# datamicroscopes/common

Measured on AMD Instinct MI355X. Metric: score_value evals/sec, higher is better.
Workload: dtype f32

## Files before the change

common_amd/csrc/abi.cpp:

```cpp
#include <algorithm>
#include <atomic>
#include <cmath>
#include <memory>
#include <mutex>
#include <new>

#include "blocked_post.hpp"
#include "launchers.hpp"
#include "linkage_host.hpp"
#include "row_range.hpp"
#include "splitmerge_math.hpp"

namespace msc {

static thread_local std::string g_last_error;

void set_error(const char *fmt, ...) {
  char buf[1024];
  va_list ap;
  va_start(ap, fmt);
  vsnprintf(buf, sizeof buf, fmt, ap);
  va_end(ap);
  g_last_error = buf;
}
// ... 1627 lines not shown
static uint64_t view_rows(const msc_state *st) {
  return st->sweep_rows_hint ? st->sweep_rows_hint : st->bound_view ? st->bound_view->nrows : 0;
}

static int refresh_fused_tables(msc_state *st) {
  const bool packed = stages_nich(st->tile_path);
  if (!st->fuse_any && !st->nich_blocks_any && !packed) return MSC_OK;
  if (launch_fuse_tables(st->ctx->stream, st->desc_fuse_dev, (int)st->fuse_split, (st->nich_blocks_any || packed) ? (int)st->fuse_nfeat : (int)st->fuse_split, st->kpad))
    return fail(MSC_EHIP, "k_fuse_tables launch failed");
  return MSC_OK;
}

static bool narrow_tail_fits(const msc_state *st) {
  const size_t nich_bytes = (size_t)(st->fuse_nfeat - st->fuse_split) * 64 * sizeof(float);
  return st->tile_narrow_tail_ok && st->K - (st->kpad - kGroupTile) <= kTailMaxGroups &&
         nich_bytes + (size_t)std::max<uint32_t>(1u, st->tail_max_rows) * kTailStride * sizeof(float) <= 64u * 1024u;
}

static int tail_plan(msc_state *st, TailPlan &tp, bool exact = true) {
  tp = TailPlan();
  tp.exact = exact;
  if (!(tp.ok = narrow_tail_fits(st))) return MSC_OK;
  MSC_HIP(grow_retained(st->retired, st->tail_pack, (size_t)st->tail_pack_rows * 64));
  tp.masked_nich = st->tail_masked_nich;
  tp.dm = st->tail_dm;
  tp.max_rows = st->tail_max_rows;
  tp.pack_rows = st->tail_pack_rows;
  tp.pack = st->tail_pack;
  return MSC_OK;
}

static bool gp_beyond_table(const msc_state *st, uint32_t f) {
  if (!st->bound_view || f >= st->bound_cols.size()) return false;
  const uint32_t c = st->bound_cols[f];
  if (is_count_family(st->feats[f].family)) return col_max_of(st, f, st->bound_view, c) >= (long long)kGpMaxTable;
  if (st->feats[f].family == MSC_DM)
    return !st->bound_view->dm_max[c].empty() && dm_max_of(st, f, st->bound_view, c, st->feats[f].dim) >= kGpMaxTable;
  return false;
}

static bool loo_needs_heavy(const msc_state *st) {
  for (uint32_t f = 0; f < st->nfeat; f++) {
    const int fam = st->feats[f].family;
    if ((is_count_family(fam) || fam == MSC_DM) && gp_beyond_table(st, f)) return true;
  }
  return false;
// ... 2438 lines not shown
```

common_amd/csrc/kernels_score.hip:

```cpp
#include <cstdlib>
#include <type_traits>

#include "commit_ops.hpp"
#include "family_math.hpp"
#include "launchers.hpp"
#include "score_block.hpp"

namespace msc {

__global__ __launch_bounds__(256) void k_prepare(const FeatDesc *__restrict__ feats, uint32_t kpad) {
  const uint32_t k = blockIdx.x * 256 + threadIdx.x;
  if (k >= kpad) return;
  prepare_group(feats[blockIdx.y], k, kpad, blockIdx.z, gridDim.z);
}

__global__ __launch_bounds__(256) void k_dm_prepare(const FeatDesc *__restrict__ feats, int f, uint32_t kpad) {
  const FeatDesc fd = feats[f];
  const uint32_t k = blockIdx.x * 256 + threadIdx.x, sub = blockIdx.y;
  if (k >= kpad || fd.dm_meta == nullptr) return;
  const uint32_t first = fd.dm_meta[2 * sub], rows = fd.dm_meta[2 * sub + 1];
  float *t = fd.tab + (size_t)first * kpad + k;
  double a = 0, n = 0;
  if (sub < fd.dim) {
    a = fd.hp[sub];
// ... 890 lines not shown
    hipLaunchKernelGGL(k_loo_own<false>, dim3((unsigned)((nrows + 255) / 256)), dim3(256), 0, stream, feats_dev, nfeat,
                       K, kpad, row0, nrows, z, crp, own);
  return hipGetLastError() == hipSuccess ? 0 : -1;
}

int launch_gp_large_fix(hipStream_t stream, int num_cus, const FeatDesc *feats_dev, int f, uint32_t K,
                        uint32_t kpad, uint64_t row0, uint64_t nrows, const int32_t *z, float *out, uint64_t ld) {
  uint64_t gx = (nrows + 3) / 4;
  const uint64_t cap = (uint64_t)num_cus * 8;
  if (gx > cap) gx = cap;
  hipLaunchKernelGGL(k_gp_large_fix, dim3((unsigned)(gx ? gx : 1)), dim3(256), 0, stream, feats_dev, f, K, kpad,
                     row0, nrows, z, out, ld);
  return hipGetLastError() == hipSuccess ? 0 : -1;
}

const Nich1Shape kNich1Shapes[kNich1NumShapes] = {{4, 2}, {4, 1}, {4, 4}, {4, 6}, {4, 3}, {4, 8}, {4, 5}, {4, 12}};

constexpr int kTailRowsWaves = 8;

__host__ __device__ inline uint32_t tail_table_rows(uint32_t family, uint32_t kind, uint32_t run_clamp, uint32_t dm_rows) {
  return family == MSC_DM ? dm_rows : kind == MSC_KIND_GENERIC ? 0u : run_clamp + 1;
}

__global__ __launch_bounds__(256) void k_tail_pack(const FeatDesc *__restrict__ feats, uint32_t kpad, uint32_t k0,
                                                    float *__restrict__ pack) {
  const int f = blockIdx.x;
  uint32_t off = 0;
  for (int i = 0; i < f; i++) off += tail_table_rows(feats[i].family, feats[i].kind, feats[i].run_clamp, feats[i].dm_rows);
  const FeatDesc &fd = feats[f];
  const uint32_t first_row = is_count_family(fd.family) ? (uint32_t)GP_T0 : 0u, rows = tail_table_rows(fd.family, fd.kind, fd.run_clamp, fd.dm_rows);
  for (uint32_t e = threadIdx.x; e < rows * 64u; e += 256u) {
    const uint32_t r = e >> 6, g = e & 63u;
    pack[(size_t)(off + r) * 64 + g] = fd.tab[(size_t)(first_row + r) * kpad + k0 + g];
  }
}

template <int TGP, bool SPLIT, bool DRAW = false, bool MNICH = false, bool EST = false, bool DMF = false>
__global__ __launch_bounds__(kTailRowsWaves * 64, (MNICH || DMF) ? 2 : 4) void k_score_tail_rows(
    const FeatDesc *__restrict__ feats_g, int nfeat, int nsplit, uint32_t K, uint32_t kpad, uint32_t k0, uint64_t row0,
    uint64_t nrows, int32_t *z, const float *__restrict__ own, const float *__restrict__ crp,
    float *__restrict__ out, uint64_t ld, const float *__restrict__ pack, uint32_t cap_rows, uint32_t kend,
    const uint64_t *__restrict__ rng, uint64_t row_id0, ZeroSpans zero) {
  uint64_t seed = 0, sweep = 0;
  if (DRAW) {
    seed = rng[0];
    sweep = rng[1];
    zero_spans(zero);
  }
  extern __shared__ __attribute__((aligned(16))) float tl[];
  __shared__ __attribute__((aligned(16))) float pr[4][64];
  __shared__ __attribute__((aligned(16))) float c0s[64];
  float *const mhl = tl + (size_t)cap_rows * kTailStride;
  typedef const __attribute__((address_space(4))) FeatDesc *scalar_fd;
  typedef const __attribute__((address_space(4))) float *scalar_f;
  const scalar_fd feats = (scalar_fd)feats_g;
  const int lane = threadIdx.x & 63, wave = __builtin_amdgcn_readfirstlane(threadIdx.x >> 6);
  const bool loo = z != nullptr, pri = crp != nullptr;
  const bool vec_ok = ((ld & 3) == 0) && ((reinterpret_cast<uintptr_t>(out) & 15) == 0);
  const uint64_t rows_per_wg = (uint64_t)kTailRowsWaves * 64;
  const uint64_t nchunks = (nrows + rows_per_wg - 1) / rows_per_wg;
  if (threadIdx.x < 64) {
    float hi = 0.f, lo = 0.f, le0 = 0.f, le1 = 0.f, e0 = 0.f, e1 = 0.f;
    if (pri) {
      hi = crp[k0 + threadIdx.x];
      lo = crp[crp_lo_cnt(kpad) + k0 + threadIdx.x];
      le0 = crp[2 * (size_t)kpad];
      le1 = crp[2 * (size_t)kpad + 1];
      e0 = crp[2 * (size_t)kpad + 2];
      e1 = crp[2 * (size_t)kpad + 3];
    }
    const bool empty = __builtin_isinf(hi);
    pr[0][threadIdx.x] = !pri ? 0.f : empty ? e0 : lo;
    pr[1][threadIdx.x] = !pri ? 0.f : empty ? e1 : lo;
    pr[2][threadIdx.x] = !pri ? -0.f : empty ? le0 : hi;
    pr[3][threadIdx.x] = !pri ? -0.f : empty ? le1 : hi;
    float c0 = 0.f;
    for (int f = nsplit; f < nfeat; f++) {
      c0 += feats_g[f].tab[(size_t)NICH_C0 * kpad + k0 + threadIdx.x];
      mhl[(size_t)(f - nsplit) * 64 + threadIdx.x] = feats_g[f].tab[(size_t)NICH_MU_HI * kpad + k0 + threadIdx.x];
    }
    c0s[threadIdx.x] = c0;
  }
  __syncthreads();
  auto load_value = [&](int f, uint64_t rr) -> uint32_t {
    const int fi = f < nfeat ? f : nfeat - 1;
    const int ct = feats[fi].col_type;
    const void *col = feats[fi].col;
    const bool u8 = ct == MSC_TYPE_B || ct == MSC_TYPE_I8 || ct == MSC_TYPE_U8;
    return u8 ? (uint32_t)reinterpret_cast<const uint8_t *>(col)[rr] : reinterpret_cast<const uint32_t *>(col)[rr];
  };
  for (uint64_t chunk = blockIdx.x; chunk < nchunks; chunk += gridDim.x) {
    const uint64_t r = chunk * rows_per_wg + (uint64_t)wave * 64 + lane;
    const bool has_row = r < nrows;
    const uint64_t rr = row0 + (has_row ? r : 0);
    int gown = (loo && has_row) ? z[r] : -1;
    if ((uint32_t)gown >= K) gown = -1;
    const bool single = pri && gown >= 0 && __builtin_isinf(crp[kpad + gown]);
    const float ownv = gown >= 0 ? own[r] : 0.f;
    const float *prl = pr[single ? 1 : 0];
    float acc[TGP], accn[SPLIT ? TGP : 1];
#pragma unroll
    for (int g = 0; g < TGP; g++) acc[g] = prl[g];
    uint32_t srow = 0, off = 0;
    int stage_end = 0;
    for (int fb = 0; fb < nsplit; fb += 8) {
      uint32_t w0 = load_value(fb, rr), w1 = load_value(fb + 1, rr), w2 = load_value(fb + 2, rr), w3 = load_value(fb + 3, rr),
               w4 = load_value(fb + 4, rr), w5 = load_value(fb + 5, rr), w6 = load_value(fb + 6, rr), w7 = load_value(fb + 7, rr);
#pragma unroll 1
      for (int i = 0; i < 8; i++) {
        const int f = fb + i;
        if (f >= nsplit) break;
        if (f == stage_end) {
          srow += off;
          off = 0;
          uint32_t rows = 0;
          while (stage_end < nsplit) {
            const uint32_t rw = tail_table_rows(feats[stage_end].family, feats[stage_end].kind, feats[stage_end].run_clamp, feats[stage_end].dm_rows);
            if (rows + rw > cap_rows && rows > 0) break;
            rows += rw;
            stage_end++;
          }
          __syncthreads();
          for (uint32_t e = threadIdx.x * 4u; e < rows * 64u; e += kTailRowsWaves * 64u * 4u) {
            const float4 v = *reinterpret_cast<const float4 *>(pack + (size_t)srow * 64 + e);
            float *d = tl + (size_t)(e >> 6) * kTailStride + (e & 63u);
            d[0] = v.x; d[1] = v.y; d[2] = v.z; d[3] = v.w;
          }
          __syncthreads();
        }
        if (DMF && feats[f].family == MSC_DM) {
          const uint32_t dim = feats[f].dim;
          const uint32_t *xr = reinterpret_cast<const uint32_t *>(feats[f].col) + rr * dim;
          const uint32_t *meta = feats[f].dm_meta;
          const uint32_t tot = has_row ? feats[f].dm_tot[rr] : 0u;
          bool dead = !has_row || tot >= kGpMaxTable;
          if (feats[f].mask != nullptr)
            for (uint32_t e = 0; e < dim; e++) dead |= feats[f].mask[rr * dim + e] != 0;
#pragma unroll
          for (int gb = 0; gb < TGP; gb += 16) {
            float hi[16], lo[16];
#pragma unroll
            for (int g = 0; g < 16; g++) hi[g] = lo[g] = 0.f;
#pragma unroll 1
            for (uint32_t st = 0; st <= dim; st++) {
              const uint32_t first_row = meta[2 * st], vcap = meta[2 * st + 1];
              uint32_t v = st < dim ? xr[st] : tot;
              v = (dead || v >= vcap) ? 0u : v;
              const float *b = tl + (size_t)(off + first_row + 2u * v) * kTailStride + gb;
#pragma unroll
              for (int g = 0; g < 16; g++) {
                hi[g] += b[g];
                lo[g] += b[kTailStride + g];
              }
            }
#pragma unroll
            for (int g = 0; g < 16; g++) acc[gb + g] += hi[g] + lo[g];
          }
          off += feats[f].dm_rows;
        } else if (MNICH && feats[f].kind == MSC_KIND_GENERIC) {
          const bool masked = feats[f].mask[rr] != 0;
          const float x = __uint_as_float(w0);
          const scalar_f tab = (scalar_f)(feats[f].tab) + k0;
          typedef float f32x4s __attribute__((ext_vector_type(4)));
          typedef const volatile __attribute__((address_space(4))) f32x4s *scalar_f4;
#pragma unroll
          for (int gb = 0; gb < TGP; gb += 4) {
            const f32x4s mh = *(scalar_f4)(tab + (size_t)NICH_MU_HI * kpad + gb), ml = *(scalar_f4)(tab + (size_t)NICH_MU_LO * kpad + gb),
                         c0 = *(scalar_f4)(tab + (size_t)NICH_C0 * kpad + gb), c1l = *(scalar_f4)(tab + (size_t)NICH_C1LN2 * kpad + gb),
                         c1 = *(scalar_f4)(tab + (size_t)NICH_C1 * kpad + gb), c2 = *(scalar_f4)(tab + (size_t)NICH_C2 * kpad + gb);
#pragma unroll
            for (int j = 0; j < 4; j++) {
              const float e = acc[gb + j] + nich_eval(x, mh[j], ml[j], c0[j], c1l[j], c1[j], c2[j]);
              acc[gb + j] = masked ? acc[gb + j] : e;
            }
            __builtin_amdgcn_sched_barrier(0);
          }
        } else {
          const uint32_t rc = feats[f].run_clamp;
          const int v = (int)w0;
          const uint32_t idx = v < 0 ? 0u : ((uint32_t)v > rc ? rc : (uint32_t)v);
          const float *b = tl + (size_t)(off + idx) * kTailStride;
#pragma unroll
          for (int g = 0; g < TGP; g++) acc[g] += b[g];
          off += rc + 1;
        }
        w0 = w1; w1 = w2; w2 = w3; w3 = w4; w4 = w5; w5 = w6; w6 = w7;
      }
    }
    if (SPLIT) {
#pragma unroll
      for (int g = 0; g < TGP; g++) accn[g] = c0s[g];
    } else if (nsplit < nfeat) {
#pragma unroll
      for (int g = 0; g < TGP; g++) acc[g] += c0s[g];
    }
    bool far = false;
    const bool blocks = nsplit < nfeat && feats[nsplit].nich_info != nullptr;
    for (int fb = nsplit; blocks && fb < nfeat; fb += 8) {
      const uint32_t w0 = load_value(fb, rr), w1 = load_value(fb + 1, rr), w2 = load_value(fb + 2, rr), w3 = load_value(fb + 3, rr),
                     w4 = load_value(fb + 4, rr), w5 = load_value(fb + 5, rr), w6 = load_value(fb + 6, rr), w7 = load_value(fb + 7, rr);
      auto lim = [&](int f) { return feats[f < nfeat ? f : nfeat - 1].nich_info->xlim; };
      far |= !(__builtin_fabsf(__uint_as_float(w0)) <= lim(fb)) | !(__builtin_fabsf(__uint_as_float(w1)) <= lim(fb + 1)) |
             !(__builtin_fabsf(__uint_as_float(w2)) <= lim(fb + 2)) | !(__builtin_fabsf(__uint_as_float(w3)) <= lim(fb + 3)) |
             !(__builtin_fabsf(__uint_as_float(w4)) <= lim(fb + 4)) | !(__builtin_fabsf(__uint_as_float(w5)) <= lim(fb + 5)) |
             !(__builtin_fabsf(__uint_as_float(w6)) <= lim(fb + 6)) | !(__builtin_fabsf(__uint_as_float(w7)) <= lim(fb + 7));
    }
    auto plain_feature = [&](int f, float x) {
      const scalar_f tab = (scalar_f)(feats[f].tab) + k0;
      const float *mhf = mhl + (size_t)(f - nsplit) * 64;
      constexpr int NB = (!SPLIT || TGP <= 32) ? 8 : 4;
      typedef float f32xn __attribute__((ext_vector_type(NB)));
      typedef const volatile __attribute__((address_space(4))) f32xn *scalar_fn;
#pragma unroll
      for (int gb = 0; gb < TGP; gb += NB) {
        const f32xn ml = *(scalar_fn)(tab + (size_t)NICH_MU_LO * kpad + gb), c1l = *(scalar_fn)(tab + (size_t)NICH_C1LN2 * kpad + gb),
                    c1 = *(scalar_fn)(tab + (size_t)NICH_C1 * kpad + gb), c2 = *(scalar_fn)(tab + (size_t)NICH_C2 * kpad + gb);
#pragma unroll
        for (int j = 0; j < NB; j++) {
          float &a = SPLIT ? accn[gb + j] : acc[gb + j];
          a = nich_accum<EST>(a, x, mhf[gb + j], ml[j], c1l[j], c1[j], c2[j]);
        }
        __builtin_amdgcn_sched_barrier(0);
      }
    };
    auto product_block = [&](int f, auto mtag, const float (&x)[4]) {
      constexpr int M = decltype(mtag)::value;
      typedef float f32x4s __attribute__((ext_vector_type(4)));
      typedef const volatile __attribute__((address_space(4))) f32x4s *scalar_f4;
      scalar_f tab[M];
      const float *mhf[M];
#pragma unroll
      for (int j = 0; j < M; j++) {
        tab[j] = (scalar_f)(feats[f + j].tab) + k0;
        mhf[j] = mhl + (size_t)(f + j - nsplit) * 64;
      }
#pragma unroll
      for (int gb = 0; gb < TGP; gb += 4) {
        f32x4s ml[M], sc[M];
#pragma unroll
        for (int j = 0; j < M; j++) {
          ml[j] = *(scalar_f4)(tab[j] + (size_t)NICH_MU_LO * kpad + gb);
          sc[j] = *(scalar_f4)(tab[j] + (size_t)NICH_C2 * kpad + gb);
        }
        const f32x4s c1l = *(scalar_f4)(tab[0] + (size_t)NICH_C1LN2 * kpad + gb);
#pragma unroll
        for (int i = 0; i < 4; i++) {
          float t[M];
#pragma unroll
          for (int j = 0; j < M; j++) t[j] = nich_t(x[j], mhf[j][gb + i], ml[j][i], sc[j][i]);
          float &a = SPLIT ? accn[gb + i] : acc[gb + i];
          a = nich_block_finish<EST>(a, nich_block_product<M>(t), c1l[i]);
        }
        __builtin_amdgcn_sched_barrier(0);
      }
    };
    for (int s0 = nsplit; s0 < nfeat;) {
      const int s1 = (int)feats[s0].grp_end;
      if (blocks) {
#pragma unroll 1
        for (int M = kNichBlock; M >= 2; M--) {
          for (int f = s0; f < s1;) {
            const int len = (int)feats[f].blk_end - f;
            if (len == M && feats[f].nich_info->blk_ok != 0u) {
              const float x[4] = {__uint_as_float(load_value(f, rr)), __uint_as_float(load_value(f + 1, rr)),
                                  __uint_as_float(load_value(f + 2, rr)), __uint_as_float(load_value(f + 3, rr))};
              if (!far) {
                if (M == 2) product_block(f, std::integral_constant<int, 2>(), x);
                else if (M == 3) product_block(f, std::integral_constant<int, 3>(), x);
                else product_block(f, std::integral_constant<int, 4>(), x);
              }
            }
            f += len;
          }
        }
      }
#pragma unroll 1
      for (int f = s0; f < s1; f++) {
        const bool covered = blocks && feats[feats[f].blk_first].nich_info->blk_ok != 0u;
        const float x = __uint_as_float(load_value(f, rr));
        if (far || !covered) plain_feature(f, x);
      }
      s0 = s1;
    }
    const float *prh = pr[single ? 3 : 2];
    if (DRAW) {
      float m = -INFINITY;
#pragma unroll
      for (int g = 0; g < TGP; g++) {
        const float sg = gown == g ? ownv : (SPLIT && nsplit < nfeat ? acc[g] + accn[g] : acc[g]) + prh[g];
        acc[g] = (uint32_t)g < K ? sg : -INFINITY;
        m = fmaxf(m, acc[g]);
      }
      float total = 0.f;
#pragma unroll
      for (int g = 0; g < TGP; g++) {
        acc[g] = __builtin_amdgcn_exp2f((acc[g] - m) * 1.44269504088896340736f);
        total += acc[g];
      }
      const float dart = philox_uniform01(seed, sweep, row_id0 + r) * total;
      float c = 0.f;
      int pick = 0;
// ... 1 lines not shown
      for (int g = 0; g < TGP; g++) {
        c += acc[g];
        pick += c < dart ? 1 : 0;
      }
      if (has_row) z[r] = pick < (int)K ? pick : (int)K - 1;
      continue;
    }
#pragma unroll
    for (int q = 0; q < TGP / 4; q++) {
      float sv[4];
#pragma unroll
      for (int c = 0; c < 4; c++) {
        const int g = 4 * q + c;
        sv[c] = gown == (int)(k0 + g) ? ownv : (SPLIT && nsplit < nfeat ? acc[g] + accn[g] : acc[g]) + prh[g];
      }
      if (has_row) store_row<false>(out, ld, r, k0 + 4 * q, kend, make_float4(sv[0], sv[1], sv[2], sv[3]), vec_ok);
    }
  }
}

template <int TGP, bool SPLIT, bool DRAW, bool MNICH, bool EST, bool DMF = false>
static void launch_tail_rows_m(hipStream_t stream, unsigned grid, size_t lds, const FeatDesc *feats_dev, int nfeat, int nsplit, uint32_t K,
                               uint32_t kpad, uint32_t k0, uint64_t row0, uint64_t nrows, const int32_t *z, const float *own,
                               const float *crp, float *out, uint64_t ld, const float *pack, uint32_t cap_rows, uint32_t kend,
                               const uint64_t *rng, uint64_t row_id0, ZeroSpans zero) {
  static unsigned long long attr_devices = 0;
  if (first_use_on_device(attr_devices))
    (void)hipFuncSetAttribute(reinterpret_cast<const void *>(k_score_tail_rows<TGP, SPLIT, DRAW, MNICH, EST, DMF>), hipFuncAttributeMaxDynamicSharedMemorySize, 64 * 1024);
  hipLaunchKernelGGL((k_score_tail_rows<TGP, SPLIT, DRAW, MNICH, EST, DMF>), (note_kernel(DRAW ? 1 : 0, "k_score_tail_rows<%d, %s, %s, %s, %s, %s>", TGP, tf(SPLIT), tf(DRAW), tf(MNICH), tf(EST), tf(DMF)), dim3(grid)), dim3(kTailRowsWaves * 64), lds, stream, feats_dev, nfeat, nsplit, K, kpad, k0,
                     row0, nrows, const_cast<int32_t *>(z), own, crp, out, ld, pack, cap_rows, kend, rng, row_id0, zero);
}
template <int TGP, bool SPLIT, bool DRAW = false, bool EST = false>
static void launch_tail_rows_t(hipStream_t stream, unsigned grid, size_t lds, int mnich, const FeatDesc *feats_dev, int nfeat, int nsplit, uint32_t K,
                               uint32_t kpad, uint32_t k0, uint64_t row0, uint64_t nrows, const int32_t *z, const float *own,
                               const float *crp, float *out, uint64_t ld, const float *pack, uint32_t cap_rows, uint32_t kend,
                               const uint64_t *rng = nullptr, uint64_t row_id0 = 0, ZeroSpans zero = ZeroSpans()) {
  if (mnich == 2) launch_tail_rows_m<TGP, SPLIT, DRAW, false, EST, true>(stream, grid, lds, feats_dev, nfeat, nsplit, K, kpad, k0, row0, nrows, z, own, crp, out, ld, pack, cap_rows, kend, rng, row_id0, zero);
  else if (mnich) launch_tail_rows_m<TGP, SPLIT, DRAW, true, EST>(stream, grid, lds, feats_dev, nfeat, nsplit, K, kpad, k0, row0, nrows, z, own, crp, out, ld, pack, cap_rows, kend, rng, row_id0, zero);
  else launch_tail_rows_m<TGP, SPLIT, DRAW, false, EST>(stream, grid, lds, feats_dev, nfeat, nsplit, K, kpad, k0, row0, nrows, z, own, crp, out, ld, pack, cap_rows, kend, rng, row_id0, zero);
}

static bool tail_rows_geometry(const TailPlan &tp, int num_cus, int nfeat, int nsplit, uint64_t nrows, uint32_t &cap_rows, size_t &lds,
                               unsigned &grid) {
  if (!tp.ok || (tp.pack_rows > 0 && tp.pack == nullptr)) return false;
  const size_t nich_bytes = (size_t)(nfeat - nsplit) * 64 * sizeof(float);
  const uint32_t fit = (uint32_t)((64u * 1024u - nich_bytes) / (kTailStride * sizeof(float)));
  cap_rows = std::max<uint32_t>(1u, std::min<uint32_t>(tp.pack_rows, std::min<uint32_t>(200u, fit)));
  lds = (size_t)cap_rows * kTailStride * sizeof(float) + nich_bytes;
  const uint64_t rows_wg = (uint64_t)kTailRowsWaves * 64;
  const uint64_t tchunks = (nrows + rows_wg - 1) / rows_wg;
  grid = (unsigned)std::min<uint64_t>(tchunks ? tchunks : 1, (uint64_t)num_cus * 2);
  return true;
}

int launch_sweep_rows(hipStream_t stream, int num_cus, const TailPlan &tp, const FeatDesc *feats_dev, int nfeat, int nsplit, uint32_t K,
                      uint32_t kpad, uint64_t row0, uint64_t nrows, uint64_t row_id0, int32_t *z, const float *own, const float *crp,
                      const uint64_t *rng, ZeroSpans zero) {
  uint32_t cap_rows = 0;
  size_t lds = 0;
  unsigned grid = 0;
  if (K > 64 || crp == nullptr || !tail_rows_geometry(tp, num_cus, nfeat, nsplit, nrows, cap_rows, lds, grid)) return fail(MSC_EHIP, "launch_sweep_rows: K = %u", K);
  if (nsplit > 0) hipLaunchKernelGGL(k_tail_pack, dim3((unsigned)nsplit), dim3(256), 0, stream, feats_dev, kpad, 0u, tp.pack);
  const uint32_t tgp = (K + 15u) / 16u * 16u;
#define MSC_SWEEP_ROWS(T) launch_tail_rows_t<T, false, true, true>(stream, grid, lds, tp.dm ? 2 : tp.masked_nich ? 1 : 0, feats_dev, nfeat, nsplit, K, kpad, 0u, row0, nrows, z, own, crp, nullptr, 0, tp.pack, cap_rows, K, rng, row_id0, zero)
  if (tgp == 16) MSC_SWEEP_ROWS(16);
  else if (tgp == 32)
    launch_tail_rows_t<32, true, true, true>(stream, grid, lds, tp.dm ? 2 : tp.masked_nich ? 1 : 0, feats_dev, nfeat, nsplit, K, kpad, 0u, row0, nrows, z, own, crp, nullptr, 0, tp.pack, cap_rows, K, rng, row_id0, zero);
  else if (tgp == 48) MSC_SWEEP_ROWS(48);
  else MSC_SWEEP_ROWS(64);
#undef MSC_SWEEP_ROWS
  return launch_status("k_score_tail_rows");
}

int launch_score_tail(hipStream_t stream, int num_cus, const TailPlan &tp, const FeatDesc *feats_dev, int nfeat, int nsplit, uint32_t K,
                      uint32_t kpad, uint32_t k0, uint64_t row0, uint64_t nrows, const int32_t *z, const float *own, const float *crp,
                      float *out, uint64_t ld) {
  uint32_t cap_rows = 0;
  size_t lds = 0;
  unsigned grid = 0;
  if (K <= k0 || K - k0 > kTailMaxGroups || !tail_rows_geometry(tp, num_cus, nfeat, nsplit, nrows, cap_rows, lds, grid)) return fail(MSC_EHIP, "launch_score_tail: K = %u", K);
  if (nrows == 0) return 0;
  const uint32_t groups = K - k0, widest = tp.exact ? 32u : 64u, nblk = (groups + widest - 1) / widest;
  const uint32_t blk = ((groups + nblk - 1) / nblk + 15u) / 16u * 16u;
  for (uint32_t kb = k0; kb < K; kb += blk) {
    const uint32_t kend = std::min<uint32_t>(K, kb + blk), tgp = (kend - kb + 15u) / 16u * 16u;
    if (nsplit > 0) hipLaunchKernelGGL(k_tail_pack, dim3((unsigned)nsplit), dim3(256), 0, stream, feats_dev, kpad, kb, tp.pack);
#define MSC_TAIL_ROWS(T, S, E) launch_tail_rows_t<T, S, false, E>(stream, grid, lds, tp.dm ? 2 : tp.masked_nich ? 1 : 0, feats_dev, nfeat, nsplit, K, kpad, kb, row0, nrows, z, own, crp, out, ld, tp.pack, cap_rows, kend)
    if (tp.exact) {
      if (tgp == 16) MSC_TAIL_ROWS(16, true, false);
      else if (tgp == 32) MSC_TAIL_ROWS(32, true, false);
      else MSC_TAIL_ROWS(48, true, false);
    } else {
      if (tgp == 16) MSC_TAIL_ROWS(16, false, true);
      else if (tgp == 32) MSC_TAIL_ROWS(32, true, true);
      else if (tgp == 48) MSC_TAIL_ROWS(48, false, true);
      else MSC_TAIL_ROWS(64, false, true);
    }
#undef MSC_TAIL_ROWS
  }
  return launch_status("k_score_tail_rows");
}

template <bool LOO, bool CRP>
static int launch_score_t(hipStream_t stream, int num_cus, ScorePath path, const TailPlan &narrow_tail, const ScoreShape &shape, const FeatDesc *feats_dev,
                           int nfeat, int nsplit, uint32_t K, uint32_t kpad, uint64_t row0, uint64_t nrows,
                           const int32_t *z, const float *own, const float *crp, float *out, uint64_t ld) {
  const uint32_t ktiles = kpad / kGroupTile;
  if (path == MSC_PATH_NICH1) {
    const bool plain_stores = (shape.nich1 & 0x100) != 0;
    const int nich1_shape = shape.nich1 & 0xff;
// ... 94 lines not shown
```

common_amd/csrc/launchers.hpp:

```cpp
#pragma once
#include <algorithm>

#include "msc_internal.hpp"

namespace msc {

inline bool first_use_on_device(unsigned long long &seen) {
  int dev = 0;
  if (hipGetDevice(&dev) != hipSuccess || dev < 0 || dev > 63) return true;
  const unsigned long long bit = 1ull << dev;
  if (seen & bit) return false;
  seen |= bit;
  return true;
}

struct UnpackFeat {
  void *dst;
  uint8_t *dst_mask;
  uint32_t offset;
  uint32_t mask_offset;
  int32_t src_type, dst_type;
  uint32_t count;
  uint32_t pad;
};
// ... 20 lines not shown
int launch_set_i32(hipStream_t stream, int32_t *dst, int32_t value);
constexpr int kLooRows = 4, kLooThreads = 1024;
int launch_loo_own(hipStream_t stream, bool heavy, bool staged, const FeatDesc *feats_dev, int nfeat, uint32_t K, uint32_t kpad, uint64_t row0,
                   uint64_t nrows, const int32_t *z, const float *crp, float *own);
int launch_gp_large_fix(hipStream_t stream, int num_cus, const FeatDesc *feats_dev, int f, uint32_t K,
                        uint32_t kpad, uint64_t row0, uint64_t nrows, const int32_t *z, float *out, uint64_t ld);
struct Nich1Shape { int q, visits; };
constexpr int kNich1NumShapes = 8;
extern const Nich1Shape kNich1Shapes[kNich1NumShapes];
constexpr uint32_t kTailMaxGroups = 128;
constexpr uint64_t kNarrowMaxRows = 65536;
constexpr uint64_t kTailMinRows = 16384;
constexpr uint32_t kTailStride = 65;
inline double tile_rounds_us(uint64_t workgroups, int num_cus, bool sweep, const PlanCost &pc = PlanCost()) {
  return (sweep ? pc.sweep_round_us : pc.tile_round_us) * (double)((workgroups + (uint64_t)num_cus - 1) / (uint64_t)num_cus);
}
inline double tail_rows_us(uint32_t groups, bool exact, uint64_t nrows, int num_cus, const PlanCost &pc = PlanCost()) {
  const uint32_t widest = exact ? 32u : 64u, nblk = (groups + widest - 1) / widest;
  const uint32_t per = ((groups + nblk - 1) / nblk + 15u) / 16u * 16u;
  const double frac = (double)nrows / (1024.0 * num_cus);
  const double rounds = frac >= 1.0 ? frac : std::max(0.6, 0.4 + 0.6 * frac);
  return (double)nblk * (pc.tail_fixed_us + pc.tail_group_us * per) * rounds;
}
struct TailPlan {
  bool ok = false;
  bool exact = true;
  bool masked_nich = false;
  bool dm = false;
  uint32_t max_rows = 0;
  uint32_t pack_rows = 0;
  float *pack = nullptr;
};
int launch_score_tail(hipStream_t stream, int num_cus, const TailPlan &tp, const FeatDesc *feats_dev, int nfeat, int nsplit, uint32_t K,
                      uint32_t kpad, uint32_t k0, uint64_t row0, uint64_t nrows, const int32_t *z, const float *own, const float *crp,
                      float *out, uint64_t ld);
struct ZeroSpans {
  unsigned long long *a = nullptr;
  size_t na = 0;
  unsigned long long *b = nullptr;
  size_t nb = 0;
};
int launch_sweep_rows(hipStream_t stream, int num_cus, const TailPlan &tp, const FeatDesc *feats_dev, int nfeat, int nsplit, uint32_t K,
                      uint32_t kpad, uint64_t row0, uint64_t nrows, uint64_t row_id0, int32_t *z, const float *own, const float *crp,
                      const uint64_t *rng, ZeroSpans zero);
int launch_score_pair_tail(hipStream_t stream, int num_cus, const FeatDesc *feats_dev, int nfeat, int nsplit, uint32_t K, uint32_t kpad,
                           uint64_t row0, uint64_t nrows, const int32_t *z, const float *own, const float *crp, float *tail, uint64_t ld);
enum class LastTile { tiles, rows, pair };
struct ScoreShape { int wave_rows = 8; bool pair = false; LastTile last = LastTile::tiles; int nich1 = 0; };
int launch_score(hipStream_t stream, int num_cus, ScorePath path, const TailPlan &narrow_tail, const ScoreShape &shape, const FeatDesc *feats_dev, int nfeat, int nsplit,
                 uint32_t K, uint32_t kpad, uint64_t row0, uint64_t nrows, const int32_t *z,
                 const float *own, const float *crp, float *out, uint64_t ld);

void note_kernel(int slot, const char *fmt, ...) __attribute__((format(printf, 2, 3)));
const char *last_kernel(int slot);
// ... 276 lines not shown
```

common_amd/csrc/msc_internal.hpp:

```cpp
#pragma once

#include <hip/hip_runtime.h>

#include <cstdarg>
#include <cstdint>
#include <cstdio>
#include <cstring>
#include <string>
#include <vector>

#include "../../include/microscopes_hip.h"
#include "dev_buf.hpp"
#include "table_validity.hpp"

namespace msc {

constexpr int kWave = 64;
constexpr int kGroupTile = 256;
constexpr unsigned kMaxDDDim = 128;
constexpr int kGrpRows = 128;
constexpr unsigned kGpMaxTable = 1024;
constexpr float kNtFastGbps = 6650.f;

void set_error(const char *fmt, ...);
// ... 432 lines not shown
  uint32_t fuse_nfeat = 0, fuse_split = 0;
  bool fuse_any = false;
  msc::DevBuf<float> fuse_tab;
  msc::DevBuf<msc::FeatDesc> desc_acc_dev;
  std::vector<msc::FeatDesc> desc_acc_host;
  msc::DevBuf<msc::NichPlanInfo> nich_info;
  msc::DevBuf<float> rn_pack;
  msc::DevBuf<msc::NichPos> rn_pos;
  bool nich_blocks_any = false;
  const msc_dataview *bound_view = nullptr;
  uint64_t bound_serial = 0;
  std::vector<uint32_t> bound_cols;
  msc::Retired retired;
  msc::DevBuf<float> scratch;
  msc::DevBuf<float> tail_scores;
  msc::DevBuf<float> own;
  msc::ScorePath tile_path = msc::MSC_PATH_TILE;
  msc::PlanCost plan_cost;
  bool tile_narrow_tail_ok = false;
  uint32_t tail_max_rows = 0, tail_pack_rows = 0;
  bool tail_masked_nich = false;
  bool tail_dm = false;
  msc::DevBuf<float> tail_pack;
  uint32_t loo_staged = 0;
  msc::DevBuf<double> marg_norm;
  msc::DevBuf<float> rows_table;
  msc::DevBuf<uint32_t> colmax_dev;
  msc::DevBuf<uint64_t> rng_dev;
  uint64_t rng_seed = 0, rng_sweep = 0;
  bool rng_valid = false;
  bool rng_bump_pending = false;
  uint64_t rng_next_sweep = 0;
  struct StepGraph {
    hipGraphExec_t exec = nullptr;
    const void *view = nullptr, *z = nullptr;
    uint64_t view_serial = 0, row0 = 0, nrows = 0, row_id0 = 0;
    float alpha = 0.f;
    std::vector<uint32_t> cols;
    msc::TableValidity::Snapshot flags;
    int seen = 0;
    bool disabled = false;
    uint64_t n_eager = 0, n_replayed = 0;
  } step_graph;
  msc::DevBuf<double> niw_qown;
  msc::DevBuf<int32_t> one_z;
  msc::DevBuf<uint32_t> niw_scratch;
// ... 49 lines not shown
```

Before: 1724 billion.

## Precompute compact per-feature tail plan records and narrow packed tables to group width

Measured after the change: 1608 billion. -6.7%, worse.

```diff
diff --git a/common_amd/csrc/abi.cpp b/common_amd/csrc/abi.cpp
--- a/common_amd/csrc/abi.cpp
+++ b/common_amd/csrc/abi.cpp
@@ -1673,6 +1673,8 @@
   tp.exact = exact;
   if (!(tp.ok = narrow_tail_fits(st))) return MSC_OK;
   MSC_HIP(grow_retained(st->retired, st->tail_pack, (size_t)st->tail_pack_rows * 64));
+  MSC_HIP(grow_retained(st->retired, st->tail_feats, tail_plan_words(st->fuse_nfeat, st->fuse_split)));
+  tp.feat_plan = st->tail_feats;
   tp.masked_nich = st->tail_masked_nich;
   tp.dm = st->tail_dm;
   tp.max_rows = st->tail_max_rows;
diff --git a/common_amd/csrc/kernels_score.hip b/common_amd/csrc/kernels_score.hip
--- a/common_amd/csrc/kernels_score.hip
+++ b/common_amd/csrc/kernels_score.hip
@@ -936,16 +936,72 @@
   return family == MSC_DM ? dm_rows : kind == MSC_KIND_GENERIC ? 0u : run_clamp + 1;
 }
 
-__global__ __launch_bounds__(256) void k_tail_pack(const FeatDesc *__restrict__ feats, uint32_t kpad, uint32_t k0,
-                                                    float *__restrict__ pack) {
+constexpr int kTailPlanTile = 1024;
+__device__ void tail_plan_records(const FeatDesc *__restrict__ feats, int nfeat, int nsplit, uint32_t cap_rows, uint32_t *__restrict__ plan) {
+  __shared__ uint32_t rws[kTailPlanTile];
+  TailFeat *const rec = reinterpret_cast<TailFeat *>(plan);
+  TailStage *const stg = reinterpret_cast<TailStage *>(rec + nfeat + kTailFeatPad);
+  const bool blocks = nsplit < nfeat && feats[nsplit].nich_info != nullptr;
+  uint32_t nst = 0, rows = 0, total = 0;
+  for (int base = 0; base < nsplit; base += kTailPlanTile) {
+    const int n = min(nsplit - base, kTailPlanTile);
+    for (int i = threadIdx.x; i < n; i += blockDim.x) {
+      const FeatDesc &fd = feats[base + i];
+      rws[i] = tail_table_rows(fd.family, fd.kind, fd.run_clamp, fd.dm_rows);
+    }
+    __syncthreads();
+    if (threadIdx.x == 0)
+      for (int i = 0; i < n; i++) {
+        const uint32_t rw = rws[i];
+        if (base + i == 0 || (rows + rw > cap_rows && rows > 0)) {
+          if (nst) stg[nst].rows = rows;
+          stg[++nst] = TailStage{(uint32_t)(base + i), total, 0u, 0u};
+          rows = 0;
+          rws[i] = kTailMetaStage;
+        } else {
+          rws[i] = rows;
+        }
+        rows += rw;
+        total += rw;
+      }
+    __syncthreads();
+    for (int i = threadIdx.x; i < n; i += blockDim.x) {
+      const FeatDesc &fd = feats[base + i];
+      const bool u8 = fd.col_type == MSC_TYPE_B || fd.col_type == MSC_TYPE_I8 || fd.col_type == MSC_TYPE_U8;
+      const bool dm = fd.family == MSC_DM, nich = !dm && fd.kind == MSC_KIND_GENERIC;
+      rec[base + i] = TailFeat{fd.col, dm ? fd.dm_rows : fd.run_clamp,
+                               rws[i] | (u8 ? kTailMetaByte : 0u) | (nich ? kTailMetaNich : 0u) | (dm ? kTailMetaDm : 0u), fd.tab, 0u, 0u};
+    }
+    __syncthreads();
+  }
+  if (threadIdx.x == 0) {
+    if (nst) stg[nst].rows = rows;
+    stg[0] = TailStage{nst, blocks ? 1u : 0u, 0u, 0u};
+    if (nst == 1) rec[0].meta &= ~kTailMetaStage;
+  }
+  for (int f = nsplit + (int)threadIdx.x; f < nfeat; f += blockDim.x) {
+    const FeatDesc &fd = feats[f];
+    const bool u8 = fd.col_type == MSC_TYPE_B || fd.col_type == MSC_TYPE_I8 || fd.col_type == MSC_TYPE_U8;
+    uint32_t blk = (fd.blk_end - (uint32_t)f) & kTailBlkLenMask;
+    if (blocks && fd.nich_info->blk_ok != 0u) blk |= kTailBlkOne;
+    if (blocks && feats[fd.blk_first].nich_info->blk_ok != 0u) blk |= kTailBlkCovered;
+    rec[f] = TailFeat{fd.col, __float_as_uint(blocks ? fd.nich_info->xlim : INFINITY), (u8 ? kTailMetaByte : 0u) | kTailMetaNich, fd.tab, fd.grp_end, blk};
+  }
+  __syncthreads();
+  if (nfeat > 0 && threadIdx.x < kTailFeatPad) rec[nfeat + threadIdx.x] = rec[nfeat - 1];
+}
+
+__global__ __launch_bounds__(256) void k_tail_pack(const FeatDesc *__restrict__ feats, int nfeat, int nsplit, uint32_t kpad, uint32_t k0,
+                                                    uint32_t width, uint32_t cap_rows, float *__restrict__ pack, uint32_t *__restrict__ plan) {
   const int f = blockIdx.x;
+  if (f == nsplit) return tail_plan_records(feats, nfeat, nsplit, cap_rows, plan);
   uint32_t off = 0;
   for (int i = 0; i < f; i++) off += tail_table_rows(feats[i].family, feats[i].kind, feats[i].run_clamp, feats[i].dm_rows);
   const FeatDesc &fd = feats[f];
   const uint32_t first_row = is_count_family(fd.family) ? (uint32_t)GP_T0 : 0u, rows = tail_table_rows(fd.family, fd.kind, fd.run_clamp, fd.dm_rows);
   for (uint32_t e = threadIdx.x; e < rows * 64u; e += 256u) {
     const uint32_t r = e >> 6, g = e & 63u;
-    pack[(size_t)(off + r) * 64 + g] = fd.tab[(size_t)(first_row + r) * kpad + k0 + g];
+    if (g < width) pack[(size_t)(off + r) * width + g] = fd.tab[(size_t)(first_row + r) * kpad + k0 + g];
   }
 }
 
@@ -953,21 +1009,36 @@
 __global__ __launch_bounds__(kTailRowsWaves * 64, (MNICH || DMF) ? 2 : 4) void k_score_tail_rows(
     const FeatDesc *__restrict__ feats_g, int nfeat, int nsplit, uint32_t K, uint32_t kpad, uint32_t k0, uint64_t row0,
     uint64_t nrows, int32_t *z, const float *__restrict__ own, const float *__restrict__ crp,
-    float *__restrict__ out, uint64_t ld, const float *__restrict__ pack, uint32_t cap_rows, uint32_t kend,
-    const uint64_t *__restrict__ rng, uint64_t row_id0, ZeroSpans zero) {
+    float *__restrict__ out, uint64_t ld, const float *__restrict__ pack, const uint32_t *__restrict__ plan_g, uint32_t cap_rows,
+    uint32_t kend, const uint64_t *__restrict__ rng, uint64_t row_id0, ZeroSpans zero) {
   uint64_t seed = 0, sweep = 0;
   if (DRAW) {
     seed = rng[0];
     sweep = rng[1];
     zero_spans(zero);
   }
+  constexpr uint32_t kStride = TGP + 1;
   extern __shared__ __attribute__((aligned(16))) float tl[];
   __shared__ __attribute__((aligned(16))) float pr[4][64];
   __shared__ __attribute__((aligned(16))) float c0s[64];
-  float *const mhl = tl + (size_t)cap_rows * kTailStride;
+  float *const mhl = tl + (size_t)cap_rows * kStride;
   typedef const __attribute__((address_space(4))) FeatDesc *scalar_fd;
   typedef const __attribute__((address_space(4))) float *scalar_f;
+  typedef const __attribute__((address_space(4))) TailFeat *scalar_tf;
+  typedef const __attribute__((address_space(4))) TailStage *scalar_ts;
   const scalar_fd feats = (scalar_fd)feats_g;
+  const scalar_tf recs = (scalar_tf)plan_g;
+  const scalar_ts stages = (scalar_ts)(recs + nfeat + kTailFeatPad);
+  const bool blocks = stages[0].row0 != 0u;
+  auto stage_in = [&](uint32_t prow, uint32_t rows) {
+    for (uint32_t e = threadIdx.x * 4u; e < rows * (uint32_t)TGP; e += kTailRowsWaves * 64u * 4u) {
+      const float4 v = *reinterpret_cast<const float4 *>(pack + (size_t)prow * TGP + e);
+      const uint32_t row = e / (uint32_t)TGP;
+      float *d = tl + row * kStride + (e - row * (uint32_t)TGP);
+      d[0] = v.x; d[1] = v.y; d[2] = v.z; d[3] = v.w;
+    }
+  };
+  if (stages[0].feat0 == 1u) stage_in(0u, stages[1].rows);
   const int lane = threadIdx.x & 63, wave = __builtin_amdgcn_readfirstlane(threadIdx.x >> 6);
   const bool loo = z != nullptr, pri = crp != nullptr;
   const bool vec_ok = ((ld & 3) == 0) && ((reinterpret_cast<uintptr_t>(out) & 15) == 0);
@@ -997,11 +1068,8 @@
   }
   __syncthreads();
   auto load_value = [&](int f, uint64_t rr) -> uint32_t {
-    const int fi = f < nfeat ? f : nfeat - 1;
-    const int ct = feats[fi].col_type;
-    const void *col = feats[fi].col;
-    const bool u8 = ct == MSC_TYPE_B || ct == MSC_TYPE_I8 || ct == MSC_TYPE_U8;
-    return u8 ? (uint32_t)reinterpret_cast<const uint8_t *>(col)[rr] : reinterpret_cast<const uint32_t *>(col)[rr];
+    const void *col = recs[f].col;
+    return (recs[f].meta & kTailMetaByte) ? (uint32_t)reinterpret_cast<const uint8_t *>(col)[rr] : reinterpret_cast<const uint32_t *>(col)[rr];
   };
   for (uint64_t chunk = blockIdx.x; chunk < nchunks; chunk += gridDim.x) {
     const uint64_t r = chunk * rows_per_wg + (uint64_t)wave * 64 + lane;
@@ -1015,8 +1083,7 @@
     float acc[TGP], accn[SPLIT ? TGP : 1];
 #pragma unroll
     for (int g = 0; g < TGP; g++) acc[g] = prl[g];
-    uint32_t srow = 0, off = 0;
-    int stage_end = 0;
+    uint32_t stg = 0;
     for (int fb = 0; fb < nsplit; fb += 8) {
       uint32_t w0 = load_value(fb, rr), w1 = load_value(fb + 1, rr), w2 = load_value(fb + 2, rr), w3 = load_value(fb + 3, rr),
                w4 = load_value(fb + 4, rr), w5 = load_value(fb + 5, rr), w6 = load_value(fb + 6, rr), w7 = load_value(fb + 7, rr);
@@ -1024,25 +1091,14 @@
       for (int i = 0; i < 8; i++) {
         const int f = fb + i;
         if (f >= nsplit) break;
-        if (f == stage_end) {
-          srow += off;
-          off = 0;
-          uint32_t rows = 0;
-          while (stage_end < nsplit) {
-            const uint32_t rw = tail_table_rows(feats[stage_end].family, feats[stage_end].kind, feats[stage_end].run_clamp, feats[stage_end].dm_rows);
-            if (rows + rw > cap_rows && rows > 0) break;
-            rows += rw;
-            stage_end++;
-          }
+        const uint32_t lim = recs[f].lim, meta = recs[f].meta, off = meta & kTailMetaRowMask;
+        if (meta & kTailMetaStage) {
+          stg++;
           __syncthreads();
-          for (uint32_t e = threadIdx.x * 4u; e < rows * 64u; e += kTailRowsWaves * 64u * 4u) {
-            const float4 v = *reinterpret_cast<const float4 *>(pack + (size_t)srow * 64 + e);
-            float *d = tl + (size_t)(e >> 6) * kTailStride + (e & 63u);
-            d[0] = v.x; d[1] = v.y; d[2] = v.z; d[3] = v.w;
-          }
+          stage_in(stages[stg].row0, stages[stg].rows);
           __syncthreads();
         }
-        if (DMF && feats[f].family == MSC_DM) {
+        if (DMF && (meta & kTailMetaDm)) {
           const uint32_t dim = feats[f].dim;
           const uint32_t *xr = reinterpret_cast<const uint32_t *>(feats[f].col) + rr * dim;
           const uint32_t *meta = feats[f].dm_meta;
@@ -1060,21 +1116,20 @@
               const uint32_t first_row = meta[2 * st], vcap = meta[2 * st + 1];
               uint32_t v = st < dim ? xr[st] : tot;
               v = (dead || v >= vcap) ? 0u : v;
-              const float *b = tl + (size_t)(off + first_row + 2u * v) * kTailStride + gb;
+              const float *b = tl + (off + first_row + 2u * v) * kStride + gb;
 #pragma unroll
               for (int g = 0; g < 16; g++) {
                 hi[g] += b[g];
-                lo[g] += b[kTailStride + g];
+                lo[g] += b[kStride + g];
               }
             }
 #pragma unroll
             for (int g = 0; g < 16; g++) acc[gb + g] += hi[g] + lo[g];
           }
-          off += feats[f].dm_rows;
-        } else if (MNICH && feats[f].kind == MSC_KIND_GENERIC) {
+        } else if (MNICH && (meta & kTailMetaNich)) {
           const bool masked = feats[f].mask[rr] != 0;
           const float x = __uint_as_float(w0);
-          const scalar_f tab = (scalar_f)(feats[f].tab) + k0;
+          const scalar_f tab = (scalar_f)(recs[f].tab) + k0;
           typedef float f32x4s __attribute__((ext_vector_type(4)));
           typedef const volatile __attribute__((address_space(4))) f32x4s *scalar_f4;
 #pragma unroll
@@ -1090,13 +1145,11 @@
             __builtin_amdgcn_sched_barrier(0);
           }
         } else {
-          const uint32_t rc = feats[f].run_clamp;
           const int v = (int)w0;
-          const uint32_t idx = v < 0 ? 0u : ((uint32_t)v > rc ? rc : (uint32_t)v);
-          const float *b = tl + (size_t)(off + idx) * kTailStride;
+          const uint32_t idx = v < 0 ? 0u : ((uint32_t)v > lim ? lim : (uint32_t)v);
+          const float *b = tl + (off + idx) * kStride;
 #pragma unroll
           for (int g = 0; g < TGP; g++) acc[g] += b[g];
-          off += rc + 1;
         }
         w0 = w1; w1 = w2; w2 = w3; w3 = w4; w4 = w5; w5 = w6; w6 = w7;
       }
@@ -1109,18 +1162,17 @@
       for (int g = 0; g < TGP; g++) acc[g] += c0s[g];
     }
     bool far = false;
-    const bool blocks = nsplit < nfeat && feats[nsplit].nich_info != nullptr;
     for (int fb = nsplit; blocks && fb < nfeat; fb += 8) {
       const uint32_t w0 = load_value(fb, rr), w1 = load_value(fb + 1, rr), w2 = load_value(fb + 2, rr), w3 = load_value(fb + 3, rr),
                      w4 = load_value(fb + 4, rr), w5 = load_value(fb + 5, rr), w6 = load_value(fb + 6, rr), w7 = load_value(fb + 7, rr);
-      auto lim = [&](int f) { return feats[f < nfeat ? f : nfeat - 1].nich_info->xlim; };
+      auto lim = [&](int f) { return __uint_as_float(recs[f].lim); };
       far |= !(__builtin_fabsf(__uint_as_float(w0)) <= lim(fb)) | !(__builtin_fabsf(__uint_as_float(w1)) <= lim(fb + 1)) |
              !(__builtin_fabsf(__uint_as_float(w2)) <= lim(fb + 2)) | !(__builtin_fabsf(__uint_as_float(w3)) <= lim(fb + 3)) |
              !(__builtin_fabsf(__uint_as_float(w4)) <= lim(fb + 4)) | !(__builtin_fabsf(__uint_as_float(w5)) <= lim(fb + 5)) |
              !(__builtin_fabsf(__uint_as_float(w6)) <= lim(fb + 6)) | !(__builtin_fabsf(__uint_as_float(w7)) <= lim(fb + 7));
     }
     auto plain_feature = [&](int f, float x) {
-      const scalar_f tab = (scalar_f)(feats[f].tab) + k0;
+      const scalar_f tab = (scalar_f)(recs[f].tab) + k0;
       const float *mhf = mhl + (size_t)(f - nsplit) * 64;
       constexpr int NB = (!SPLIT || TGP <= 32) ? 8 : 4;
       typedef float f32xn __attribute__((ext_vector_type(NB)));
@@ -1145,7 +1197,7 @@
       const float *mhf[M];
 #pragma unroll
       for (int j = 0; j < M; j++) {
-        tab[j] = (scalar_f)(feats[f + j].tab) + k0;
+        tab[j] = (scalar_f)(recs[f + j].tab) + k0;
         mhf[j] = mhl + (size_t)(f + j - nsplit) * 64;
       }
 #pragma unroll
@@ -1169,13 +1221,14 @@
       }
     };
     for (int s0 = nsplit; s0 < nfeat;) {
-      const int s1 = (int)feats[s0].grp_end;
+      const int s1 = (int)recs[s0].grp_end;
       if (blocks) {
 #pragma unroll 1
         for (int M = kNichBlock; M >= 2; M--) {
           for (int f = s0; f < s1;) {
-            const int len = (int)feats[f].blk_end - f;
-            if (len == M && feats[f].nich_info->blk_ok != 0u) {
+            const uint32_t blk = recs[f].blk;
+            const int len = (int)(blk & kTailBlkLenMask);
+            if (len == M && (blk & kTailBlkOne)) {
               const float x[4] = {__uint_as_float(load_value(f, rr)), __uint_as_float(load_value(f + 1, rr)),
                                   __uint_as_float(load_value(f + 2, rr)), __uint_as_float(load_value(f + 3, rr))};
               if (!far) {
@@ -1190,7 +1243,7 @@
       }
 #pragma unroll 1
       for (int f = s0; f < s1; f++) {
-        const bool covered = blocks && feats[feats[f].blk_first].nich_info->blk_ok != 0u;
+        const bool covered = (recs[f].blk & kTailBlkCovered) != 0u;
         const float x = __uint_as_float(load_value(f, rr));
         if (far || !covered) plain_feature(f, x);
       }
@@ -1238,31 +1291,31 @@
 template <int TGP, bool SPLIT, bool DRAW, bool MNICH, bool EST, bool DMF = false>
 static void launch_tail_rows_m(hipStream_t stream, unsigned grid, size_t lds, const FeatDesc *feats_dev, int nfeat, int nsplit, uint32_t K,
                                uint32_t kpad, uint32_t k0, uint64_t row0, uint64_t nrows, const int32_t *z, const float *own,
-                               const float *crp, float *out, uint64_t ld, const float *pack, uint32_t cap_rows, uint32_t kend,
+                               const float *crp, float *out, uint64_t ld, const float *pack, const uint32_t *plan, uint32_t cap_rows, uint32_t kend,
                                const uint64_t *rng, uint64_t row_id0, ZeroSpans zero) {
   static unsigned long long attr_devices = 0;
   if (first_use_on_device(attr_devices))
     (void)hipFuncSetAttribute(reinterpret_cast<const void *>(k_score_tail_rows<TGP, SPLIT, DRAW, MNICH, EST, DMF>), hipFuncAttributeMaxDynamicSharedMemorySize, 64 * 1024);
   hipLaunchKernelGGL((k_score_tail_rows<TGP, SPLIT, DRAW, MNICH, EST, DMF>), (note_kernel(DRAW ? 1 : 0, "k_score_tail_rows<%d, %s, %s, %s, %s, %s>", TGP, tf(SPLIT), tf(DRAW), tf(MNICH), tf(EST), tf(DMF)), dim3(grid)), dim3(kTailRowsWaves * 64), lds, stream, feats_dev, nfeat, nsplit, K, kpad, k0,
-                     row0, nrows, const_cast<int32_t *>(z), own, crp, out, ld, pack, cap_rows, kend, rng, row_id0, zero);
+                     row0, nrows, const_cast<int32_t *>(z), own, crp, out, ld, pack, plan, cap_rows, kend, rng, row_id0, zero);
 }
 template <int TGP, bool SPLIT, bool DRAW = false, bool EST = false>
 static void launch_tail_rows_t(hipStream_t stream, unsigned grid, size_t lds, int mnich, const FeatDesc *feats_dev, int nfeat, int nsplit, uint32_t K,
                                uint32_t kpad, uint32_t k0, uint64_t row0, uint64_t nrows, const int32_t *z, const float *own,
-                               const float *crp, float *out, uint64_t ld, const float *pack, uint32_t cap_rows, uint32_t kend,
+                               const float *crp, float *out, uint64_t ld, const float *pack, const uint32_t *plan, uint32_t cap_rows, uint32_t kend,
                                const uint64_t *rng = nullptr, uint64_t row_id0 = 0, ZeroSpans zero = ZeroSpans()) {
-  if (mnich == 2) launch_tail_rows_m<TGP, SPLIT, DRAW, false, EST, true>(stream, grid, lds, feats_dev, nfeat, nsplit, K, kpad, k0, row0, nrows, z, own, crp, out, ld, pack, cap_rows, kend, rng, row_id0, zero);
-  else if (mnich) launch_tail_rows_m<TGP, SPLIT, DRAW, true, EST>(stream, grid, lds, feats_dev, nfeat, nsplit, K, kpad, k0, row0, nrows, z, own, crp, out, ld, pack, cap_rows, kend, rng, row_id0, zero);
-  else launch_tail_rows_m<TGP, SPLIT, DRAW, false, EST>(stream, grid, lds, feats_dev, nfeat, nsplit, K, kpad, k0, row0, nrows, z, own, crp, out, ld, pack, cap_rows, kend, rng, row_id0, zero);
-}
-
-static bool tail_rows_geometry(const TailPlan &tp, int num_cus, int nfeat, int nsplit, uint64_t nrows, uint32_t &cap_rows, size_t &lds,
-                               unsigned &grid) {
-  if (!tp.ok || (tp.pack_rows > 0 && tp.pack == nullptr)) return false;
+  if (mnich == 2) launch_tail_rows_m<TGP, SPLIT, DRAW, false, EST, true>(stream, grid, lds, feats_dev, nfeat, nsplit, K, kpad, k0, row0, nrows, z, own, crp, out, ld, pack, plan, cap_rows, kend, rng, row_id0, zero);
+  else if (mnich) launch_tail_rows_m<TGP, SPLIT, DRAW, true, EST>(stream, grid, lds, feats_dev, nfeat, nsplit, K, kpad, k0, row0, nrows, z, own, crp, out, ld, pack, plan, cap_rows, kend, rng, row_id0, zero);
+  else launch_tail_rows_m<TGP, SPLIT, DRAW, false, EST>(stream, grid, lds, feats_dev, nfeat, nsplit, K, kpad, k0, row0, nrows, z, own, crp, out, ld, pack, plan, cap_rows, kend, rng, row_id0, zero);
+}
+
+static bool tail_rows_geometry(const TailPlan &tp, int num_cus, int nfeat, int nsplit, uint64_t nrows, uint32_t width, uint32_t &cap_rows,
+                               size_t &lds, unsigned &grid) {
+  if (!tp.ok || (tp.pack_rows > 0 && tp.pack == nullptr) || tp.feat_plan == nullptr) return false;
   const size_t nich_bytes = (size_t)(nfeat - nsplit) * 64 * sizeof(float);
-  const uint32_t fit = (uint32_t)((64u * 1024u - nich_bytes) / (kTailStride * sizeof(float)));
-  cap_rows = std::max<uint32_t>(1u, std::min<uint32_t>(tp.pack_rows, std::min<uint32_t>(200u, fit)));
-  lds = (size_t)cap_rows * kTailStride * sizeof(float) + nich_bytes;
+  const uint32_t fit = (uint32_t)((64u * 1024u - nich_bytes) / ((width + 1) * sizeof(float)));
+  cap_rows = std::max<uint32_t>(1u, std::min<uint32_t>(tp.pack_rows, fit));
+  lds = (size_t)cap_rows * (width + 1) * sizeof(float) + nich_bytes;
   const uint64_t rows_wg = (uint64_t)kTailRowsWaves * 64;
   const uint64_t tchunks = (nrows + rows_wg - 1) / rows_wg;
   grid = (unsigned)std::min<uint64_t>(tchunks ? tchunks : 1, (uint64_t)num_cus * 2);
@@ -1275,13 +1328,13 @@
   uint32_t cap_rows = 0;
   size_t lds = 0;
   unsigned grid = 0;
-  if (K > 64 || crp == nullptr || !tail_rows_geometry(tp, num_cus, nfeat, nsplit, nrows, cap_rows, lds, grid)) return fail(MSC_EHIP, "launch_sweep_rows: K = %u", K);
-  if (nsplit > 0) hipLaunchKernelGGL(k_tail_pack, dim3((unsigned)nsplit), dim3(256), 0, stream, feats_dev, kpad, 0u, tp.pack);
   const uint32_t tgp = (K + 15u) / 16u * 16u;
-#define MSC_SWEEP_ROWS(T) launch_tail_rows_t<T, false, true, true>(stream, grid, lds, tp.dm ? 2 : tp.masked_nich ? 1 : 0, feats_dev, nfeat, nsplit, K, kpad, 0u, row0, nrows, z, own, crp, nullptr, 0, tp.pack, cap_rows, K, rng, row_id0, zero)
+  if (K > 64 || crp == nullptr || !tail_rows_geometry(tp, num_cus, nfeat, nsplit, nrows, tgp, cap_rows, lds, grid)) return fail(MSC_EHIP, "launch_sweep_rows: K = %u", K);
+  hipLaunchKernelGGL(k_tail_pack, dim3((unsigned)nsplit + 1), dim3(256), 0, stream, feats_dev, nfeat, nsplit, kpad, 0u, tgp, cap_rows, tp.pack, tp.feat_plan);
+#define MSC_SWEEP_ROWS(T) launch_tail_rows_t<T, false, true, true>(stream, grid, lds, tp.dm ? 2 : tp.masked_nich ? 1 : 0, feats_dev, nfeat, nsplit, K, kpad, 0u, row0, nrows, z, own, crp, nullptr, 0, tp.pack, tp.feat_plan, cap_rows, K, rng, row_id0, zero)
   if (tgp == 16) MSC_SWEEP_ROWS(16);
   else if (tgp == 32)
-    launch_tail_rows_t<32, true, true, true>(stream, grid, lds, tp.dm ? 2 : tp.masked_nich ? 1 : 0, feats_dev, nfeat, nsplit, K, kpad, 0u, row0, nrows, z, own, crp, nullptr, 0, tp.pack, cap_rows, K, rng, row_id0, zero);
+    launch_tail_rows_t<32, true, true, true>(stream, grid, lds, tp.dm ? 2 : tp.masked_nich ? 1 : 0, feats_dev, nfeat, nsplit, K, kpad, 0u, row0, nrows, z, own, crp, nullptr, 0, tp.pack, tp.feat_plan, cap_rows, K, rng, row_id0, zero);
   else if (tgp == 48) MSC_SWEEP_ROWS(48);
   else MSC_SWEEP_ROWS(64);
 #undef MSC_SWEEP_ROWS
@@ -1294,14 +1347,15 @@
   uint32_t cap_rows = 0;
   size_t lds = 0;
   unsigned grid = 0;
-  if (K <= k0 || K - k0 > kTailMaxGroups || !tail_rows_geometry(tp, num_cus, nfeat, nsplit, nrows, cap_rows, lds, grid)) return fail(MSC_EHIP, "launch_score_tail: K = %u", K);
+  if (K <= k0 || K - k0 > kTailMaxGroups || !tail_rows_geometry(tp, num_cus, nfeat, nsplit, nrows, 64u, cap_rows, lds, grid)) return fail(MSC_EHIP, "launch_score_tail: K = %u", K);
   if (nrows == 0) return 0;
   const uint32_t groups = K - k0, widest = tp.exact ? 32u : 64u, nblk = (groups + widest - 1) / widest;
   const uint32_t blk = ((groups + nblk - 1) / nblk + 15u) / 16u * 16u;
   for (uint32_t kb = k0; kb < K; kb += blk) {
     const uint32_t kend = std::min<uint32_t>(K, kb + blk), tgp = (kend - kb + 15u) / 16u * 16u;
-    if (nsplit > 0) hipLaunchKernelGGL(k_tail_pack, dim3((unsigned)nsplit), dim3(256), 0, stream, feats_dev, kpad, kb, tp.pack);
-#define MSC_TAIL_ROWS(T, S, E) launch_tail_rows_t<T, S, false, E>(stream, grid, lds, tp.dm ? 2 : tp.masked_nich ? 1 : 0, feats_dev, nfeat, nsplit, K, kpad, kb, row0, nrows, z, own, crp, out, ld, tp.pack, cap_rows, kend)
+    (void)tail_rows_geometry(tp, num_cus, nfeat, nsplit, nrows, tgp, cap_rows, lds, grid);
+    hipLaunchKernelGGL(k_tail_pack, dim3((unsigned)nsplit + 1), dim3(256), 0, stream, feats_dev, nfeat, nsplit, kpad, kb, tgp, cap_rows, tp.pack, tp.feat_plan);
+#define MSC_TAIL_ROWS(T, S, E) launch_tail_rows_t<T, S, false, E>(stream, grid, lds, tp.dm ? 2 : tp.masked_nich ? 1 : 0, feats_dev, nfeat, nsplit, K, kpad, kb, row0, nrows, z, own, crp, out, ld, tp.pack, tp.feat_plan, cap_rows, kend)
     if (tp.exact) {
       if (tgp == 16) MSC_TAIL_ROWS(16, true, false);
       else if (tgp == 32) MSC_TAIL_ROWS(32, true, false);
diff --git a/common_amd/csrc/launchers.hpp b/common_amd/csrc/launchers.hpp
--- a/common_amd/csrc/launchers.hpp
+++ b/common_amd/csrc/launchers.hpp
@@ -66,6 +66,24 @@
   const double rounds = frac >= 1.0 ? frac : std::max(0.6, 0.4 + 0.6 * frac);
   return (double)nblk * (pc.tail_fixed_us + pc.tail_group_us * per) * rounds;
 }
+struct alignas(32) TailFeat {
+  const void *col;
+  uint32_t lim;
+  uint32_t meta;
+  const float *tab;
+  uint32_t grp_end;
+  uint32_t blk;
+};
+constexpr uint32_t kTailFeatPad = 8;
+constexpr uint32_t kTailMetaRowMask = 0xffffu, kTailMetaByte = 1u << 16, kTailMetaNich = 1u << 17, kTailMetaDm = 1u << 18,
+                   kTailMetaStage = 1u << 19;
+constexpr uint32_t kTailBlkLenMask = 0xffu,
+                   kTailBlkOne = 1u << 8,
+                   kTailBlkCovered = 1u << 9;
+struct alignas(16) TailStage { uint32_t feat0, row0, rows, pad; };
+inline size_t tail_plan_words(uint32_t nfeat, uint32_t nsplit) {
+  return ((size_t)(nfeat + kTailFeatPad) * sizeof(TailFeat) + (size_t)(nsplit + 1) * sizeof(TailStage)) / sizeof(uint32_t);
+}
 struct TailPlan {
   bool ok = false;
   bool exact = true;
@@ -74,6 +92,7 @@
   uint32_t max_rows = 0;
   uint32_t pack_rows = 0;
   float *pack = nullptr;
+  uint32_t *feat_plan = nullptr;
 };
 int launch_score_tail(hipStream_t stream, int num_cus, const TailPlan &tp, const FeatDesc *feats_dev, int nfeat, int nsplit, uint32_t K,
                       uint32_t kpad, uint32_t k0, uint64_t row0, uint64_t nrows, const int32_t *z, const float *own, const float *crp,
diff --git a/common_amd/csrc/msc_internal.hpp b/common_amd/csrc/msc_internal.hpp
--- a/common_amd/csrc/msc_internal.hpp
+++ b/common_amd/csrc/msc_internal.hpp
@@ -478,6 +478,7 @@
   bool tail_masked_nich = false;
   bool tail_dm = false;
   msc::DevBuf<float> tail_pack;
+  msc::DevBuf<uint32_t> tail_feats;
   uint32_t loo_staged = 0;
   msc::DevBuf<double> marg_norm;
   msc::DevBuf<float> rows_table;
```
